# google/TensorNetwork

Hardware: NVIDIA H100
Metric: pairwise contractions/s (higher is better)
Workload: dtype bf16

## Files before the change

include/tnb200.h:

```cpp
#ifndef TNB200_H_
#define TNB200_H_

#include <stdint.h>

#if defined(TNB200_BUILD)
#define TNB200_API __attribute__((visibility("default")))
#else
#define TNB200_API
#endif

#ifdef __cplusplus
extern "C" {
#endif

#define TNB200_MAX_NDIM 16
#define TNB200_ABI_VERSION 1

typedef enum {
  TNB200_OK = 0,
  TNB200_ERR_INVALID = -1,
  TNB200_ERR_DTYPE = -2,
  TNB200_ERR_CUDA = -3,
  TNB200_ERR_UNSUPPORTED = -4,
  TNB200_ERR_NOCONV = -5
// ... 76 lines not shown
                     int32_t axis1, int32_t axis2, void* stream);
TNB200_API int32_t tnb200_diagflat(const tnb200_tensor_t* a, const tnb200_tensor_t* c, int64_t k,
                        void* stream);

TNB200_API int32_t tnb200_svd(const tnb200_tensor_t* a, const tnb200_tensor_t* u, const tnb200_tensor_t* s,
                   const tnb200_tensor_t* vh, int32_t* info_dev, void* stream);
TNB200_API int32_t tnb200_svd_truncation_count(const tnb200_tensor_t* s, int64_t max_singular_values,
                                    int32_t use_error, double max_truncation_error,
                                    int32_t relative, int64_t* keep_dev, void* stream);

TNB200_API int32_t tnb200_eigh(const tnb200_tensor_t* a, const tnb200_tensor_t* w, const tnb200_tensor_t* v,
                               int32_t* info_dev, void* stream);

TNB200_API int32_t tnb200_arnoldi_orth(const tnb200_tensor_t* v, int32_t j, const tnb200_tensor_t* w, void* h_dev,
                                       void* stream);

TNB200_API int32_t tnb200_qr(const tnb200_tensor_t* a, const tnb200_tensor_t* q, const tnb200_tensor_t* r,
                  int32_t non_negative_diagonal, void* stream);

TNB200_API int32_t tnb200_lu_factor(const tnb200_tensor_t* a, const tnb200_tensor_t* lu, int32_t* piv_dev,
                                    int32_t* info_dev, void* stream);
TNB200_API int32_t tnb200_inv(const tnb200_tensor_t* a, const tnb200_tensor_t* x, int32_t* info_dev, void* stream);

TNB200_API int32_t tnb200_blocksparse_tensordot(const void* a_data, const void* b_data, void* c_data,
                                     int32_t dtype, int32_t nsect, const int64_t* dims_dev,
                                     const int64_t* a_map_dev, const int64_t* a_off_dev,
                                     const int64_t* b_map_dev, const int64_t* b_off_dev,
                                     const int64_t* c_map_dev, const int64_t* c_off_dev,
                                     int64_t max_m, int64_t max_n, int32_t conj_b, void* stream);

TNB200_API int32_t tnb200_svd_batched(const void* a_data, int32_t dtype, int32_t nprob, const int64_t* dims_dev,
                                      const int64_t* a_off_dev, void* u_data, const int64_t* u_off_dev, void* s_data,
                                      const int64_t* s_off_dev, void* vh_data, const int64_t* vh_off_dev,
                                      int64_t max_m, int64_t max_n, int32_t* status_dev, void* stream);

TNB200_API int32_t tnb200_blocksparse_maps(int32_t nlegs, const int64_t* dims, const int64_t* charges_dev, const int64_t* leg_off,
                                           const int32_t* order, int32_t partition, int32_t split, int64_t modulus, int64_t shift,
                                           int32_t nbins, const int64_t* tables_dev, int64_t nnz, int64_t* map_dev, void* stream);

TNB200_API int32_t tnb200_gather(const void* src, const int64_t* idx_dev, void* dst, int64_t n, int32_t dtype,
                                 int32_t scatter, void* stream);

typedef struct {
  tnb200_tensor_t a, b, c;
  int32_t naxes, nbatch;
  int32_t axes_a[TNB200_MAX_NDIM], axes_b[TNB200_MAX_NDIM];
  int32_t batch_a[TNB200_MAX_NDIM], batch_b[TNB200_MAX_NDIM];
  int32_t dep_a, dep_b;
} tnb200_chain_step_t;
TNB200_API int32_t tnb200_chain_create(int32_t nsteps, const tnb200_chain_step_t* steps, int32_t* first_unsupported,
                                       void** handle);
TNB200_API int32_t tnb200_chain_launch(void* handle, void* stream);
TNB200_API int32_t tnb200_chain_destroy(void* handle);

TNB200_API int32_t tnb200_thin_run_create(int32_t nsteps, const tnb200_chain_step_t* steps, int32_t* first_unsupported,
                                          void** handle);
TNB200_API int32_t tnb200_thin_run_launch(void* handle, void* stream);
TNB200_API int32_t tnb200_thin_run_destroy(void* handle);

#ifdef __cplusplus
}
#endif
#endif
```

tensornetwork_b200/_lib.py:

```python
import ctypes
import os

MAX_NDIM = 16
LIB_PATH = os.path.join(os.path.dirname(os.path.abspath(__file__)), "lib", "libtnb200.so")

F64, F32, F16, BF16, C64, C128, I32, I64, BOOL = range(9)
OK, ERR_INVALID, ERR_DTYPE, ERR_CUDA, ERR_UNSUPPORTED, ERR_NOCONV = 0, -1, -2, -3, -4, -5
ADD, SUB, MUL, DIV, POW = range(5)
CONJ, SQRT, ABS, NEG, EXP, LOG, SIN, COS, SIGN, REAL, IMAG = range(11)
LT, LE, GT, GE = range(4)
CONJ_A, CONJ_B = 1, 2
MATH_DEFAULT, MATH_STRICT, MATH_SIMT = 0 << 4, 1 << 4, 2 << 4


class TensorDesc(ctypes.Structure):
  _fields_ = [("data", ctypes.c_void_p), ("dtype", ctypes.c_int32), ("ndim", ctypes.c_int32),
              ("shape", ctypes.c_int64 * MAX_NDIM), ("stride", ctypes.c_int64 * MAX_NDIM)]


class ChainStep(ctypes.Structure):
  _fields_ = [("a", TensorDesc), ("b", TensorDesc), ("c", TensorDesc), ("naxes", ctypes.c_int32), ("nbatch", ctypes.c_int32),
              ("axes_a", ctypes.c_int32 * MAX_NDIM), ("axes_b", ctypes.c_int32 * MAX_NDIM),
              ("batch_a", ctypes.c_int32 * MAX_NDIM), ("batch_b", ctypes.c_int32 * MAX_NDIM),
              ("dep_a", ctypes.c_int32), ("dep_b", ctypes.c_int32)]


_P = ctypes.POINTER(TensorDesc)
_i32, _i64, _u64, _dbl, _vp = (ctypes.c_int32, ctypes.c_int64, ctypes.c_uint64, ctypes.c_double,
                               ctypes.c_void_p)
_pi32 = ctypes.POINTER(ctypes.c_int32)

SIGNATURES = {
    "tnb200_last_error": (ctypes.c_char_p, []),
    "tnb200_abi_version": (_i32, []),
    "tnb200_device_info": (_i32, [_pi32, _pi32, _pi32, ctypes.POINTER(_i64)]),
    "tnb200_last_kernel": (ctypes.c_char_p, []),
    "tnb200_launch_count": (_i64, []),
    "tnb200_tensordot": (_i32, [_P, _P, _P, _i32, _pi32, _pi32, _i32, _pi32, _pi32, _i32, _vp]),
    "tnb200_copy": (_i32, [_P, _P, _i32, _vp]),
    "tnb200_binary": (_i32, [_i32, _P, _P, _P, _vp]),
    "tnb200_unary": (_i32, [_i32, _P, _P, _vp]),
    "tnb200_affine_inplace": (_i32, [_P, _dbl, _dbl, _dbl, _dbl, _vp]),
    "tnb200_scale_by_device_scalar": (_i32, [_P, _vp, _i32, _i32, _vp]),
    "tnb200_axpy": (_i32, [_P, _P, _dbl, _dbl, _vp, _dbl, _vp]),
    "tnb200_fill": (_i32, [_P, _dbl, _dbl, _vp]),
    "tnb200_compare": (_i32, [_i32, _P, _P, _P, _vp]),
    "tnb200_index_update": (_i32, [_P, _P, _dbl, _dbl, _vp, _i32, _P, _vp]),
    "tnb200_eye": (_i32, [_P, _i64, _vp]),
    "tnb200_randn": (_i32, [_P, _u64, _vp]),
    "tnb200_uniform": (_i32, [_P, _dbl, _dbl, _u64, _vp]),
    "tnb200_norm": (_i32, [_P, _vp, _vp]),
    "tnb200_dot": (_i32, [_P, _P, _i32, _vp, _vp]),
    "tnb200_sum": (_i32, [_P, _P, _i32, _pi32, _vp]),
    "tnb200_trace": (_i32, [_P, _P, _i64, _i32, _i32, _vp]),
    "tnb200_diagflat": (_i32, [_P, _P, _i64, _vp]),
    "tnb200_svd": (_i32, [_P, _P, _P, _P, _vp, _vp]),
    "tnb200_svd_truncation_count": (_i32, [_P, _i64, _i32, _dbl, _i32, _vp, _vp]),
    "tnb200_eigh": (_i32, [_P, _P, _P, _vp, _vp]),
    "tnb200_arnoldi_orth": (_i32, [_P, _i32, _P, _vp, _vp]),
    "tnb200_qr": (_i32, [_P, _P, _P, _i32, _vp]),
    "tnb200_lu_factor": (_i32, [_P, _P, _vp, _vp, _vp]),
    "tnb200_inv": (_i32, [_P, _P, _vp, _vp]),
    "tnb200_blocksparse_maps": (_i32, [_i32, _vp, _vp, _vp, _vp, _i32, _i32, _i64, _i64, _i32, _vp, _i64, _vp, _vp]),
    "tnb200_svd_batched": (_i32, [_vp, _i32, _i32, _vp, _vp, _vp, _vp, _vp, _vp, _vp, _vp, _i64, _i64, _vp, _vp]),
    "tnb200_gather": (_i32, [_vp, _vp, _vp, _i64, _i32, _i32, _vp]),
    "tnb200_blocksparse_tensordot": (_i32, [_vp, _vp, _vp, _i32, _i32, _vp, _vp, _vp, _vp, _vp,
                                            _vp, _vp, _i64, _i64, _i32, _vp]),
    "tnb200_chain_create": (_i32, [_i32, ctypes.POINTER(ChainStep), _pi32, ctypes.POINTER(_vp)]),
    "tnb200_chain_launch": (_i32, [_vp, _vp]),
    "tnb200_chain_destroy": (_i32, [_vp]),
    "tnb200_thin_run_create": (_i32, [_i32, ctypes.POINTER(ChainStep), _pi32, ctypes.POINTER(_vp)]),
    "tnb200_thin_run_launch": (_i32, [_vp, _vp]),
    "tnb200_thin_run_destroy": (_i32, [_vp]),
}

_lib = None


def load(path=None):
  global _lib
  if _lib is not None:
    return _lib
  path = path or os.environ.get("TNB200_LIB", LIB_PATH)
  if not os.path.exists(path):
    raise OSError("libtnb200.so not found at {} — build it with "
                  "`python -m tensornetwork_b200.build` (there is no CPU fallback)".format(path))
  lib = ctypes.CDLL(path)
  for name, (res, args) in SIGNATURES.items():
    fn = getattr(lib, name)
    fn.restype = res
    fn.argtypes = args
  if lib.tnb200_abi_version() != 1:
    raise OSError("libtnb200.so ABI version mismatch")
  _lib = lib
  return lib


def set_lib(obj):
  global _lib
  _lib = obj


class Tnb200Error(RuntimeError):
  pass


def check(rc):
  if rc == 0:
    return
  msg = _lib.tnb200_last_error()
  msg = msg.decode() if isinstance(msg, bytes) else str(msg)
  if rc == ERR_INVALID:
    raise ValueError(msg)
  if rc == ERR_DTYPE:
    raise TypeError(msg)
  if rc == ERR_UNSUPPORTED:
    raise NotImplementedError(msg)
  raise Tnb200Error("tnb200 status {}: {}".format(rc, msg))
```

tensornetwork_b200/csrc/gemm_wgmma.cu:

```cuda
#include "gemm.cuh"
#include "wgmma.cuh"
#include <cuda.h>
#include <mutex>
#include <vector>

namespace tnb {

__device__ __forceinline__ uint32_t smem_u32(const void* p) { return (uint32_t)__cvta_generic_to_shared(p); }

__device__ __forceinline__ void mbar_init(uint32_t bar, uint32_t count) {
  asm volatile("mbarrier.init.shared::cta.b64 [%0], %1;" ::"r"(bar), "r"(count));
}
__device__ __forceinline__ void mbar_expect_tx(uint32_t bar, uint32_t bytes) {
  asm volatile("mbarrier.arrive.expect_tx.shared::cta.b64 _, [%0], %1;" ::"r"(bar), "r"(bytes) : "memory");
}
__device__ __forceinline__ void mbar_arrive(uint32_t bar) {
  asm volatile("mbarrier.arrive.shared::cta.b64 _, [%0];" ::"r"(bar) : "memory");
}
__device__ __forceinline__ void mbar_wait(uint32_t bar, uint32_t parity) {
  uint32_t done = 0;
#pragma unroll 1
  for (uint32_t it = 0; it < (1u << 28); ++it) {
    asm volatile(
        "{\n\t.reg .pred p;\n\t"
        "mbarrier.try_wait.parity.shared::cta.b64 p, [%1], %2;\n\t"
        "selp.u32 %0, 1, 0, p;\n\t}"
        : "=r"(done) : "r"(bar), "r"(parity) : "memory");
    if (done) return;
  }
  __trap();
}
__device__ __forceinline__ void tma_load_5d(uint32_t dst, const CUtensorMap* map, uint32_t bar, int c0, int c1, int c2, int c3, int c4) {
  asm volatile(
      "cp.async.bulk.tensor.5d.shared::cluster.global.mbarrier::complete_tx::bytes [%0], [%1, {%3, %4, %5, %6, %7}], [%2];"
      ::"r"(dst), "l"(map), "r"(bar), "r"(c0), "r"(c1), "r"(c2), "r"(c3), "r"(c4) : "memory");
}
__device__ __forceinline__ void tma_load_5d_pair(uint32_t dst, const CUtensorMap* map, uint32_t bar,
                                                 int c0, int c1, int c2, int c3, int c4) {
  asm volatile(
      "cp.async.bulk.tensor.5d.shared::cluster.global.mbarrier::complete_tx::bytes.multicast::cluster"
      " [%0], [%1, {%3, %4, %5, %6, %7}], [%2], %8;"
      ::"r"(dst), "l"(map), "r"(bar), "r"(c0), "r"(c1), "r"(c2), "r"(c3), "r"(c4), "h"((uint16_t)0x3) : "memory");
}
__device__ __forceinline__ uint32_t cluster_ctarank() {
  uint32_t r;
  asm volatile("mov.u32 %0, %%cluster_ctarank;" : "=r"(r));
  return r;
}
__device__ __forceinline__ void mbar_arrive_cluster(uint32_t bar, uint32_t cta) {
  asm volatile(
      "{\n\t.reg .b32 remote;\n\t"
      "mapa.shared::cluster.u32 remote, %0, %1;\n\t"
      "mbarrier.arrive.shared::cluster.b64 _, [remote];\n\t}"
      ::"r"(bar), "r"(cta) : "memory");
}
// ... 23 lines not shown
}

struct TcParams {
  int64_t M, N, K, batch;
  int BN, num_kb, stages, out_kind;
  int64_t tiles_m, tiles_n, num_tiles;
  int a_mn, b_mn;
  uint32_t a_fe, a_ke, b_fe, b_ke;
  void* C; int64_t c_sm, c_sb;
  int64_t c_cs;
  int vec_ok;
};

constexpr int kBM = 128;
constexpr int kRowBytes = 128;
constexpr int kThreads = 384;

struct alignas(64) ChainStepDev {
  CUtensorMap tmA, tmB, tmC;
  TcParams p;
  int dep_a, dep_b;
  uint32_t need_a, need_b;
  int tiles_per_sample;
};
struct ChainSeg { long long tile0; int step, sample0, nsamples, pad; };
struct ChainParams {
  const ChainStepDev* steps;
  const ChainSeg* segs;
  uint32_t* done;
  long long num_tiles;
  int nsegs, batch, stages, stage_bytes;
};
constexpr int kConsumerWarps = 8;
constexpr int kChainBN16 = 256, kChainBN32 = 128;
constexpr int kBoxBytes = 64 * 128;
constexpr int kChainStageHalf = 2 * kBoxBytes;

struct KernelArgs {
  CUtensorMap tmA, tmB;
  TcParams p;
  ChainParams cp;
  int stage_bytes;
};

__device__ __forceinline__ uint32_t ld_acquire_u32(const uint32_t* p) {
  uint32_t v;
  asm volatile("ld.acquire.gpu.global.u32 %0, [%1];" : "=r"(v) : "l"(p) : "memory");
  return v;
}
__device__ __forceinline__ void red_release_add_u32(uint32_t* p, uint32_t v) {
  asm volatile("red.release.gpu.global.add.u32 [%0], %1;" ::"l"(p), "r"(v) : "memory");
}
#ifdef TNB200_CHAIN_PHASES
constexpr int kPhases = 6;
constexpr int kPhaseCtas = 1024;
__device__ unsigned long long g_chain_phase[kPhaseCtas * kPhases];
__device__ __forceinline__ unsigned long long phase_clock() {
  unsigned long long t;
  asm volatile("mov.u64 %0, %%globaltimer;" : "=l"(t)::"memory");
  return t;
}
#define TNB_PHASE(...) __VA_ARGS__
#define TNB_PHASE_ADD(slot, v) (g_chain_phase[blockIdx.x * kPhases + (slot)] += (v))
#else
#define TNB_PHASE(...)
#endif

__device__ __forceinline__ void chain_wait(const uint32_t* ctr, uint32_t need) {
#pragma unroll 1
  for (uint32_t it = 0; it < (1u << 24); ++it) {
    if (ld_acquire_u32(ctr) >= need) return;
    __nanosleep(64);
  }
  __trap();
}

struct Tile {
  const TcParams* p;
  const CUtensorMap *ma, *mb;
  const ChainStepDev* sd;
  int bi, mi, ni, step;
  bool live;
};
template <bool CHAIN>
__device__ __forceinline__ void decode_tile(const KernelArgs& a, long long tile, int rank, int& cursor, Tile& t) {
  if (!CHAIN) {
    uint32_t x = (uint32_t)tile;
    const uint32_t tn = (uint32_t)a.p.tiles_n, tm = (uint32_t)a.p.tiles_m;
    t.ni = (int)(x % tn); x /= tn;
    t.mi = (int)(x % tm);
    t.bi = (int)(x / tm);
    t.p = &a.p; t.ma = &a.tmA; t.mb = &a.tmB; t.sd = nullptr; t.step = 0;
    t.live = true;
  } else {
    const ChainParams& cp = a.cp;
    while (cursor + 1 < cp.nsegs && tile >= cp.segs[cursor + 1].tile0) ++cursor;
    const ChainSeg sg = cp.segs[cursor];
    const ChainStepDev* sd = cp.steps + sg.step;
    uint32_t local = (uint32_t)(tile - sg.tile0);
    const uint32_t tn = (uint32_t)sd->p.tiles_n, tm = (uint32_t)sd->p.tiles_m, pm = (tm + 1) / 2;
    t.ni = (int)(local % tn); local /= tn;
    t.mi = 2 * (int)(local % pm) + rank;
    t.bi = sg.sample0 + (int)(local / pm);
    t.step = sg.step;
    t.p = &sd->p; t.ma = &sd->tmA; t.mb = &sd->tmB; t.sd = sd;
    t.live = (uint32_t)t.mi < tm;
  }
// ... 8 lines not shown
    const int m = idx & 31, rest = idx >> 5, kc = rest & 7;
    const int r = (rest >> 3) * 32 + m;
    const bool is_a = r < rows_a;
    const int rr = is_a ? r : r - rows_a;
    const uint32_t src = staging + (is_a ? 0u : a_bytes) + (uint32_t)(rr >> 5) * 4096u;
    const uint32_t dst = stage + (is_a ? 0u : a_bytes) + (uint32_t)rr * 128u + (uint32_t)((kc ^ (rr & 7)) << 4);
    uint32_t v[4];
#pragma unroll
    for (int i = 0; i < 4; ++i) {
      const int k = kc * 4 + i;
      const uint32_t addr = src + (uint32_t)k * 128u + (uint32_t)((((m >> 2) ^ (k & 7)) << 4) | ((m & 3) << 2));
      asm volatile("ld.shared.b32 %0, [%1];" : "=r"(v[i]) : "r"(addr) : "memory");
    }
    asm volatile("st.shared.v4.b32 [%0], {%1, %2, %3, %4};" ::"r"(dst), "r"(v[0]), "r"(v[1]), "r"(v[2]), "r"(v[3]) : "memory");
  }
  asm volatile("fence.proxy.async.shared::cta;" ::: "memory");
}

template <int KIND, int BN, int TA, int TB>
__device__ __forceinline__ void mma_k(float* d, uint64_t a, uint64_t b, uint32_t acc) {
  if constexpr (KIND == 2) {
    if constexpr (BN == 64) wgmma_n64_tf32(d, a, b, acc);
    else if constexpr (BN == 128) wgmma_n128_tf32(d, a, b, acc);
    else wgmma_n256_tf32(d, a, b, acc);
  } else if constexpr (KIND == 0) {
    if constexpr (BN == 64) wgmma_n64_bf16<TA, TB>(d, a, b, acc);
    else if constexpr (BN == 128) wgmma_n128_bf16<TA, TB>(d, a, b, acc);
    else wgmma_n256_bf16<TA, TB>(d, a, b, acc);
  } else {
    if constexpr (BN == 64) wgmma_n64_f16<TA, TB>(d, a, b, acc);
    else if constexpr (BN == 128) wgmma_n128_f16<TA, TB>(d, a, b, acc);
    else wgmma_n256_f16<TA, TB>(d, a, b, acc);
  }
}

template <bool PAIR>
__device__ __forceinline__ void release_slot(uint32_t bar) {
  if constexpr (PAIR) { mbar_arrive_cluster(bar, 0); mbar_arrive_cluster(bar, 1); }
  else mbar_arrive(bar);
}

__device__ __forceinline__ void drainloop(int S, uint32_t bar_base, int num_kb, int lane, int& s, uint32_t& ph) {
#pragma unroll 1
  for (int kb = 0; kb < num_kb; ++kb) {
    mbar_wait(bar_base + 8u * s, ph);
    __syncwarp();
    if (lane == 0) release_slot<true>(bar_base + 8u * (S + s));
    if (++s == S) { s = 0; ph ^= 1; }
  }
}

template <int KIND, int BN, int TA, int TB, bool PAIR>
__device__ __forceinline__ void mainloop(float* d, uint8_t* smem, int stage_bytes, int S, uint32_t bar_base, int num_kb,
                                         int a_mn, int b_mn, int wg, int ctid, int lane, int& s, uint32_t& ph) {
  constexpr int BK = kRowBytes / (KIND == 2 ? 4 : 2);
  constexpr uint32_t a_lbo = TA ? BK * kRowBytes : 16u, b_lbo = TB ? BK * kRowBytes : 16u;
  constexpr uint32_t a_kstep = TA ? 16u * kRowBytes : 32u, b_kstep = TB ? 16u * kRowBytes : 32u;
  int prev = -1;
  for (int kb = 0; kb < num_kb; ++kb) {
    TNB_PHASE(const unsigned long long tw = phase_clock();)
    mbar_wait(bar_base + 8u * s, ph);
    TNB_PHASE(if (ctid == 0) TNB_PHASE_ADD(1, phase_clock() - tw);)
    const uint32_t sa = smem_u32(smem + (size_t)s * stage_bytes);
    if (KIND == 2 && (a_mn || b_mn)) {
      transpose_stage_tf32(sa, a_mn, b_mn, BN, ctid);
      consumers_sync();
    }
    const uint32_t sa_wg = sa + (uint32_t)wg * 64u * kRowBytes;
    const uint32_t sb = sa + kBM * kRowBytes;
    wg_fence();
#pragma unroll
    for (int k = 0; k < 4; ++k)
      mma_k<KIND, BN, TA, TB>(d, gmma_desc(sa_wg + k * a_kstep, a_lbo, 1024u), gmma_desc(sb + k * b_kstep, b_lbo, 1024u),
                              (kb > 0 || k > 0) ? 1u : 0u);
    wg_commit();
    if (prev >= 0) {
      wg_wait<1>();
      __syncwarp();
      if (lane == 0) release_slot<PAIR>(bar_base + 8u * (S + prev));
    }
    prev = s;
    if (++s == S) { s = 0; ph ^= 1; }
  }
  wg_wait<0>();
  __syncwarp();
  if (lane == 0) release_slot<PAIR>(bar_base + 8u * (S + prev));
}

__device__ __forceinline__ void store_one(const TcParams& p, int64_t off, float v) {
  if (p.out_kind == 2) ((float*)p.C)[off] = v;
  else if (p.out_kind == 0) ((__nv_bfloat16*)p.C)[off] = __float2bfloat16_rn(v);
  else ((__half*)p.C)[off] = __float2half_rn(v);
}
__device__ __forceinline__ void store_pair(const TcParams& p, int64_t off, float v0, float v1) {
  if (p.out_kind == 2) *(float2*)((float*)p.C + off) = make_float2(v0, v1);
  else if (p.out_kind == 0) *(__nv_bfloat162*)((__nv_bfloat16*)p.C + off) = __floats2bfloat162_rn(v0, v1);
  else *(__half2*)((__half*)p.C + off) = __floats2half2_rn(v0, v1);
}

template <int KIND, int BN, bool CHAIN>
__global__ void __launch_bounds__(kThreads, 1)
gemm_wgmma_kernel(const __grid_constant__ KernelArgs args) {
  constexpr int ES = KIND == 2 ? 4 : 2;
  constexpr int BK = kRowBytes / ES;
  constexpr int CHUNK = kRowBytes / ES;
  constexpr int A_BYTES = kBM * kRowBytes;
  constexpr int B_BYTES = BN * kRowBytes;
  extern __shared__ __align__(1024) uint8_t smem_raw[];
  uint8_t* smem = (uint8_t*)(((uintptr_t)smem_raw + 1023) & ~(uintptr_t)1023);
  const int STAGE_BYTES = args.stage_bytes;
  const int S = CHAIN ? args.cp.stages : args.p.stages;
  const long long num_tiles = CHAIN ? args.cp.num_tiles : args.p.num_tiles;
  constexpr int STAGE_HALF = kChainStageHalf;
  const uint32_t staging = smem_u32(smem + (size_t)S * STAGE_BYTES);
  uint64_t* bars = (uint64_t*)(smem + (size_t)S * STAGE_BYTES + (CHAIN ? 2 * STAGE_HALF : 0));
// ... 3 lines not shown
  auto staged_bar = [&](int wg) { return bar_base + 8u * (2 * S + wg); };
  auto freed_bar = [&](int wg) { return bar_base + 8u * (2 * S + 2 + wg); };

  const int warp = threadIdx.x >> 5, lane = threadIdx.x & 31;
  TNB_PHASE(const unsigned long long t_start = phase_clock();)
  if (threadIdx.x == 0) {
    if (!CHAIN) {
      asm volatile("prefetch.tensormap [%0];" ::"l"(&args.tmA) : "memory");
      asm volatile("prefetch.tensormap [%0];" ::"l"(&args.tmB) : "memory");
    }
    for (int s = 0; s < S; ++s) {
      mbar_init(full_bar(s), 1);
      mbar_init(empty_bar(s), (CHAIN ? 2 : 1) * kConsumerWarps);
    }
    if (CHAIN)
      for (int wg = 0; wg < 2; ++wg) { mbar_init(staged_bar(wg), 4); mbar_init(freed_bar(wg), 1); }
    asm volatile("fence.mbarrier_init.release.cluster;" ::: "memory");
  }
  if constexpr (CHAIN) cluster_sync();
  else __syncthreads();
  const int rank = CHAIN ? (int)cluster_ctarank() : 0;
  const long long first = CHAIN ? blockIdx.x / 2 : blockIdx.x, step = CHAIN ? gridDim.x / 2 : gridDim.x;

  if (warp == 0) {
    constexpr int B_SPLIT = CHAIN ? 2 : 1;
    int s = 0; uint32_t ph = 0;
    int cursor = 0;
    for (long long tile = first; tile < num_tiles; tile += step) {
      Tile t;
      decode_tile<CHAIN>(args, tile, rank, cursor, t);
      const TcParams& p = *t.p;
      const int a_mn = p.a_mn, b_mn = p.b_mn;
      const int nA = t.live ? (a_mn ? kBM / CHUNK : 1) : 0;
      const int nB = b_mn ? BN / CHUNK / B_SPLIT : 1;
      const bool mine = lane < nA + nB;
      const bool is_a = lane < nA;
      const bool mn = is_a ? (a_mn != 0) : (b_mn != 0);
      const int c = is_a ? lane : rank * nB + lane - nA;
      const int fbox = mn ? CHUNK : (is_a ? kBM : BN / B_SPLIT);
      const uint32_t fe = is_a ? p.a_fe : p.b_fe, ke = is_a ? p.a_ke : p.b_ke;
      const CUtensorMap* map = is_a ? t.ma : t.mb;
      uint32_t dst_off = (is_a ? 0u : (uint32_t)A_BYTES) + (uint32_t)(c * fbox * kRowBytes);
      if (KIND == 2 && mn) dst_off += A_BYTES + B_BYTES;
      const int f = (is_a ? t.mi * kBM : t.ni * BN) + c * fbox;
      const int f_in = fe ? (int)((uint32_t)f % fe) : f, f_out = fe ? (int)((uint32_t)f / fe) : 0;
      const uint32_t tx_bytes = (t.live ? A_BYTES : 0) + B_BYTES;
      const int num_kb = p.num_kb;
      if (CHAIN) {
        if (lane == 0) {
          TNB_PHASE(const unsigned long long tw = phase_clock();)
          const ChainStepDev* sd = t.sd;
          if (sd->dep_a >= 0) chain_wait(args.cp.done + (size_t)sd->dep_a * args.cp.batch + t.bi, sd->need_a);
          if (sd->dep_b >= 0) chain_wait(args.cp.done + (size_t)sd->dep_b * args.cp.batch + t.bi, sd->need_b);
          TNB_PHASE(TNB_PHASE_ADD(0, phase_clock() - tw);)
        }
        __syncwarp();
        asm volatile("fence.proxy.async;" ::: "memory");
      }
      int k_in = 0, k_out = 0;
      for (int kb = 0; kb < num_kb; ++kb) {
        mbar_wait(empty_bar(s), ph ^ 1);
        const uint32_t full = full_bar(s);
        if (lane == 0) mbar_expect_tx(full, tx_bytes);
        __syncwarp();
        if (mine) {
          const uint32_t dst = smem_u32(smem + (size_t)s * STAGE_BYTES) + dst_off;
          const int x0 = mn ? f_in : k_in, x1 = mn ? k_in : f_in, x2 = mn ? k_out : f_out, x3 = mn ? f_out : k_out;
          if (CHAIN && !is_a) tma_load_5d_pair(dst, map, full, x0, x1, x2, x3, t.bi);
          else                tma_load_5d(dst, map, full, x0, x1, x2, x3, t.bi);
        }
        k_in += BK;
        if (ke && (uint32_t)k_in >= ke) { k_in = 0; ++k_out; }
        if (++s == S) { s = 0; ph ^= 1; }
      }
    }
  } else if (warp >= 4) {
    const int ctid = threadIdx.x - 128;
    const int wg = ctid >> 7;
    const int wt = ctid & 127;
    int s = 0; uint32_t ph = 0;
    uint32_t eph = 0;
    int cursor = 0;
    float d[BN / 2];
    for (long long tile = first; tile < num_tiles; tile += step) {
      Tile t;
      decode_tile<CHAIN>(args, tile, rank, cursor, t);
      const TcParams& p = *t.p;
      const int a_mn = p.a_mn, b_mn = p.b_mn, num_kb = p.num_kb;
      if (CHAIN && !t.live) {
        drainloop(S, bar_base, num_kb, lane, s, ph);
        continue;
      }
      TNB_PHASE(const unsigned long long tk = phase_clock();)
      if constexpr (KIND == 2) {
        mainloop<KIND, BN, 0, 0, CHAIN>(d, smem, STAGE_BYTES, S, bar_base, num_kb, a_mn, b_mn, wg, ctid, lane, s, ph);
      } else {
        if (a_mn && b_mn) mainloop<KIND, BN, 1, 1, CHAIN>(d, smem, STAGE_BYTES, S, bar_base, num_kb, a_mn, b_mn, wg, ctid, lane, s, ph);
        else if (a_mn) mainloop<KIND, BN, 1, 0, CHAIN>(d, smem, STAGE_BYTES, S, bar_base, num_kb, a_mn, b_mn, wg, ctid, lane, s, ph);
        else if (b_mn) mainloop<KIND, BN, 0, 1, CHAIN>(d, smem, STAGE_BYTES, S, bar_base, num_kb, a_mn, b_mn, wg, ctid, lane, s, ph);
        else mainloop<KIND, BN, 0, 0, CHAIN>(d, smem, STAGE_BYTES, S, bar_base, num_kb, a_mn, b_mn, wg, ctid, lane, s, ph);
      }
      TNB_PHASE(const unsigned long long te = phase_clock(); if (ctid == 0) TNB_PHASE_ADD(2, te - tk);)
      const int r0 = (wt >> 5) * 16 + (lane >> 2);
      if constexpr (CHAIN) {
        constexpr int J_PER_PASS = BN / 8 * STAGE_HALF / (4 * kBoxBytes);
        const uint32_t half = staging + (uint32_t)wg * STAGE_HALF;
#pragma unroll
        for (int pass = 0; pass < 4 * kBoxBytes / STAGE_HALF; ++pass) {
          mbar_wait(freed_bar(wg), eph ^ 1);
#pragma unroll
          for (int jj = 0; jj < J_PER_PASS; ++jj) {
            const int j = pass * J_PER_PASS + jj;
            const uint32_t colb = (uint32_t)(8 * j + 2 * (lane & 3)) * ES - (uint32_t)pass * STAGE_HALF / 64;
#pragma unroll
            for (int h = 0; h < 2; ++h) {
              const uint32_t r = (uint32_t)(r0 + 8 * h);
              const uint32_t addr = half + (colb >> 7) * kBoxBytes + r * 128u + ((((colb >> 4) & 7) ^ (r & 7)) << 4) + (colb & 15);
              const float v0 = d[4 * j + 2 * h], v1 = d[4 * j + 2 * h + 1];
              if constexpr (KIND == 2) {
                asm volatile("st.shared.v2.f32 [%0], {%1, %2};" ::"r"(addr), "f"(v0), "f"(v1) : "memory");
              } else {
                uint32_t u;
                if constexpr (KIND == 0) { __nv_bfloat162 x = __floats2bfloat162_rn(v0, v1); u = *(uint32_t*)&x; }
                else { __half2 x = __floats2half2_rn(v0, v1); u = *(uint32_t*)&x; }
                asm volatile("st.shared.b32 [%0], %1;" ::"r"(addr), "r"(u) : "memory");
              }
            }
          }
          asm volatile("fence.proxy.async.shared::cta;" ::: "memory");
          __syncwarp();
          if (lane == 0) mbar_arrive(staged_bar(wg));
          eph ^= 1;
        }
        TNB_PHASE(if (ctid == 0) { TNB_PHASE_ADD(3, phase_clock() - te); TNB_PHASE_ADD(5, 1); })
        continue;
      }
      const int64_t row0 = (int64_t)t.mi * kBM + wg * 64 + r0;
      const int64_t n0 = (int64_t)t.ni * BN + 2 * (lane & 3);
      const int64_t cb = (int64_t)t.bi * p.c_sb;
#pragma unroll
      for (int h = 0; h < 2; ++h) {
        const int64_t row = row0 + 8 * h;
        if (row < p.M) {
#pragma unroll
          for (int j = 0; j < BN / 8; ++j) {
            const int64_t col = n0 + 8 * j;
            const float v0 = d[4 * j + 2 * h], v1 = d[4 * j + 2 * h + 1];
            if (p.c_cs == 1) {
              const int64_t off = cb + row * p.c_sm + col;
              if (p.vec_ok && col + 1 < p.N) store_pair(p, off, v0, v1);
              else {
                if (col < p.N) store_one(p, off, v0);
                if (col + 1 < p.N) store_one(p, off + 1, v1);
              }
            } else {
              const int64_t off = cb + row * p.c_sm + col * p.c_cs;
              if (col < p.N) store_one(p, off, v0);
              if (col + 1 < p.N) store_one(p, off + p.c_cs, v1);
            }
          }
        }
      }
    }
    TNB_PHASE(if (ctid == 0) TNB_PHASE_ADD(4, phase_clock() - t_start);)
  } else if (CHAIN && warp == 1 && lane == 0) {
    int cursor = 0;
    uint32_t sph = 0;
    for (long long tile = first; tile < num_tiles; tile += step) {
      Tile t;
      decode_tile<CHAIN>(args, tile, rank, cursor, t);
      if (!t.live) continue;
      const CUtensorMap* mc = &t.sd->tmC;
#pragma unroll 1
      for (int pass = 0; pass < 4 * kBoxBytes / STAGE_HALF; ++pass) {
#pragma unroll 1
        for (int wg = 0; wg < 2; ++wg) {
          mbar_wait(staged_bar(wg), sph);
          for (int b = 0; b < STAGE_HALF / kBoxBytes; ++b) {
            const int box = pass * (STAGE_HALF / kBoxBytes) + b;
            tma_store_3d(mc, staging + (uint32_t)(wg * STAGE_HALF + b * kBoxBytes), t.ni * BN + box * (128 / ES),
                         t.mi * kBM + wg * 64, t.bi);
          }
          bulk_commit();
          bulk_wait_read_all();
          mbar_arrive(freed_bar(wg));
        }
        sph ^= 1;
      }
      bulk_wait_all();
      asm volatile("fence.proxy.async.global;" ::: "memory");
      red_release_add_u32(args.cp.done + (size_t)t.step * args.cp.batch + t.bi, 1u);
    }
  }
  if constexpr (CHAIN) cluster_sync();
}

typedef CUresult (*EncodeTiledFn)(CUtensorMap*, CUtensorMapDataType, cuuint32_t, void*, const cuuint64_t*,
                                  const cuuint64_t*, const cuuint32_t*, const cuuint32_t*, CUtensorMapInterleave,
                                  CUtensorMapSwizzle, CUtensorMapL2promotion, CUtensorMapFloatOOBfill);
static EncodeTiledFn get_encode() {
  static EncodeTiledFn fn = nullptr;
  static std::once_flag once;
  std::call_once(once, []() {
    void* p = nullptr;
    cudaDriverEntryPointQueryResult q;
    if (cudaGetDriverEntryPoint("cuTensorMapEncodeTiled", &p, cudaEnableDefault, &q) == cudaSuccess &&
        q == cudaDriverEntryPointSuccess)
      fn = (EncodeTiledFn)p;
  });
  return fn;
}

static int es_of(int dt) { return dt == TNB200_F32 ? 4 : 2; }
static int kind_of(int dt) { return dt == TNB200_BF16 ? 0 : (dt == TNB200_F16 ? 1 : 2); }

static int view_major(int dtype, const OperandView& v, int64_t ext_f, int64_t ext_k, int64_t batch) {
  if (dtype != TNB200_F32 && dtype != TNB200_F16 && dtype != TNB200_BF16) return -1;
// ... 184 lines not shown
    t.c_sm = g.c_sn; t.c_sn = g.c_sm;
    return gemm_wgmma(t, st);
  }
  KernelArgs args;
  memset(&args, 0, sizeof(args));
  {
    TcPrep prep;
    int rc = tc_prepare(g, false, prep);
    if (rc) return rc;
    args.tmA = prep.tmA; args.tmB = prep.tmB; args.p = prep.p; args.stage_bytes = prep.stage_bytes;
  }
  const int kind = kind_of(g.dtype);
  KernelFn fn = kernel_of(kind, args.p.BN, false);
  static bool attr_set[3][3] = {};
  const int bi = args.p.BN == 64 ? 0 : (args.p.BN == 128 ? 1 : 2);
  if (!attr_set[kind][bi]) {
    int rc = raise_smem(fn);
    if (rc) return rc;
    attr_set[kind][bi] = true;
  }
  const int64_t sms = num_sms();
  const int64_t grid = args.p.num_tiles < sms ? args.p.num_tiles : sms;
  fn<<<(unsigned)grid, kThreads, smem_of(args.p.stages, args.stage_bytes), st>>>(args);
  TNB_LAUNCH_CHECK();
  count_launch();
  set_kernel_name(kind == 0 ? "wgmma_bf16" : (kind == 1 ? "wgmma_f16" : "wgmma_tf32"));
  return 0;
}

struct ChainHandle {
  ChainStepDev* d_steps = nullptr;
  ChainSeg* d_segs = nullptr;
  uint32_t* d_done = nullptr;
  KernelArgs args;
  int kind = 0, nsteps = 0;
  size_t smem = 0, done_bytes = 0;
  unsigned grid = 0;
};

struct PairLaunch {
  cudaLaunchAttribute attr;
  cudaLaunchConfig_t cfg;
  PairLaunch(unsigned grid, size_t smem, cudaStream_t st) {
    memset(&attr, 0, sizeof(attr));
    attr.id = cudaLaunchAttributeClusterDimension;
    attr.val.clusterDim.x = 2; attr.val.clusterDim.y = 1; attr.val.clusterDim.z = 1;
    memset(&cfg, 0, sizeof(cfg));
    cfg.gridDim = dim3(grid); cfg.blockDim = dim3(kThreads); cfg.dynamicSmemBytes = smem; cfg.stream = st;
    cfg.attrs = &attr; cfg.numAttrs = 1;
  }
  PairLaunch(const PairLaunch&) = delete;
};

int gemm_chain_create(int nsteps, const GemmProblem* probs, const int* dep_a, const int* dep_b, int* first_unsupported,
                      void** handle) {
  *handle = nullptr;
  if (nsteps < 1) return TNB200_ERR_INVALID;
  auto reject = [&](int i, int rc) { if (first_unsupported) *first_unsupported = i; return rc; };
  for (int i = 0; i < nsteps; ++i) {
    const GemmProblem& g = probs[i];
    if (g.M < 128 || g.N < 128 || g.batch != probs[0].batch || g.dtype != probs[0].dtype)
      return reject(i, TNB200_ERR_UNSUPPORTED);
  }
  const int dtype = probs[0].dtype;
  const int64_t batch = probs[0].batch;
  std::vector<ChainStepDev> steps(nsteps);
  int max_stage = 0;
  std::vector<int64_t> step_bytes(nsteps), out_bytes(nsteps);
  for (int i = 0; i < nsteps; ++i) {
    const GemmProblem& g = probs[i];
    if (g.conjA || g.conjB || g.swapped) return reject(i, TNB200_ERR_UNSUPPORTED);
    if (g.dtype != TNB200_F32 && g.dtype != TNB200_F16 && g.dtype != TNB200_BF16) return reject(i, TNB200_ERR_UNSUPPORTED);
    if (g.c_sn != 1 || g.M >= (1LL << 31) || g.N >= (1LL << 31) || g.K >= (1LL << 31)) return reject(i, TNB200_ERR_UNSUPPORTED);
    if (dep_a[i] >= i || dep_b[i] >= i) return TNB200_ERR_INVALID;
    TcPrep prep;
    int rc = tc_prepare(g, true, prep);
    if (rc) return reject(i, rc);
    ChainStepDev& sd = steps[i];
    memset(&sd, 0, sizeof(sd));
    rc = encode_output(&sd.tmC, g);
    if (rc) return reject(i, rc);
    sd.tmA = prep.tmA; sd.tmB = prep.tmB; sd.p = prep.p;
    sd.dep_a = dep_a[i]; sd.dep_b = dep_b[i];
    sd.tiles_per_sample = (int)(prep.p.tiles_m * prep.p.tiles_n);
    if (prep.stage_bytes > max_stage) max_stage = prep.stage_bytes;
    step_bytes[i] = (g.M * g.K + g.N * g.K + g.M * g.N) * es_of(dtype);
    out_bytes[i] = g.M * g.N * es_of(dtype);
  }
  for (int i = 0; i < nsteps; ++i) {
    if (steps[i].dep_a >= 0) steps[i].need_a = (uint32_t)steps[steps[i].dep_a].tiles_per_sample;
    if (steps[i].dep_b >= 0) steps[i].need_b = (uint32_t)steps[steps[i].dep_b].tiles_per_sample;
  }
  const int kind = kind_of(dtype);
  KernelFn fn = kernel_of(kind, 0, true);
  {
    static bool attr_set[3] = {};
    if (!attr_set[kind]) {
      int rc = raise_smem(fn);
      if (rc) return rc;
      attr_set[kind] = true;
    }
  }
  const int staging = 2 * kChainStageHalf;
  int stages = (227 * 1024 - 1024 - staging - 256) / max_stage;
  if (stages > 8) stages = 8;
  if (stages < 2) return TNB200_ERR_UNSUPPORTED;
  const size_t smem = smem_of(stages, max_stage) + staging + 4 * 8;
  int clusters = 0;
  {
    PairLaunch pl(2 * num_sms(), smem, nullptr);
    if (cudaOccupancyMaxActiveClusters(&clusters, (void*)fn, &pl.cfg) != cudaSuccess) {
      cudaGetLastError();
      clusters = 0;
    }
  }
  if (clusters < 1) return TNB200_ERR_UNSUPPORTED;
  std::vector<int> pps(nsteps);
  for (int i = 0; i < nsteps; ++i) pps[i] = (int)(steps[i].p.tiles_n * ((steps[i].p.tiles_m + 1) / 2));
  auto env_int = [](const char* name, int dflt) { const char* e = getenv(name); return e ? atoi(e) : dflt; };
  int min_pps = pps[0];
  for (int i = 1; i < nsteps; ++i) if (pps[i] < min_pps) min_pps = pps[i];
  if (batch * min_pps < clusters && !env_int("TNB200_CHAIN_FORCE", 0))
    return TNB200_ERR_UNSUPPORTED;
  int l2 = 0;
  {
    int dev = 0;
    if (cudaGetDevice(&dev) != cudaSuccess || cudaDeviceGetAttribute(&l2, cudaDevAttrL2CacheSize, dev) != cudaSuccess) {
      cudaGetLastError();
      l2 = 0;
    }
  }
  int g_wave = 1;
  std::vector<int> last_reader(nsteps, -1);
  for (int i = 0; i < nsteps; ++i) {
    for (const int d : {dep_a[i], dep_b[i]}) {
      if (d < 0) continue;
      last_reader[d] = i;
      int64_t gap = 0;
      for (int j = d; j < i; ++j) gap += pps[j];
      const int g = (int)((clusters + gap - 1) / gap);
      if (g > g_wave) g_wave = g;
    }
  }
  int64_t live_bytes = 0;
  for (int i = 0; i < nsteps; ++i) {
    int64_t live = step_bytes[i];
    for (int j = 0; j < i; ++j)
      if (last_reader[j] > i && dep_a[i] != j && dep_b[i] != j) live += out_bytes[j];
    if (live > live_bytes) live_bytes = live;
  }
  const int g_l2 = (int)(l2 / live_bytes);
  int G = env_int("TNB200_CHAIN_G", g_wave > g_l2 ? g_wave : g_l2);
  if (G < 1) G = 1;
  const int64_t rounds = (batch + G - 1) / G;
  std::vector<ChainSeg> segs;
  long long tile0 = 0;
  for (int64_t r = 0; r < rounds; ++r) {
    const int64_t r0 = batch * r / rounds, r1 = batch * (r + 1) / rounds;
    for (int i = 0; i < nsteps; ++i) {
      ChainSeg sg;
      sg.tile0 = tile0; sg.step = i; sg.sample0 = (int)r0; sg.nsamples = (int)(r1 - r0); sg.pad = 0;
      segs.push_back(sg);
      tile0 += (long long)(r1 - r0) * pps[i];
    }
  }
  ChainHandle* h = new ChainHandle();
  h->kind = kind;
  h->nsteps = nsteps;
  h->done_bytes = sizeof(uint32_t) * (size_t)nsteps * (size_t)batch;
  cudaError_t e = cudaMalloc(&h->d_steps, sizeof(ChainStepDev) * steps.size());
  if (e == cudaSuccess) e = cudaMalloc(&h->d_segs, sizeof(ChainSeg) * segs.size());
  if (e == cudaSuccess) e = cudaMalloc(&h->d_done, h->done_bytes);
  if (e == cudaSuccess) e = cudaMemcpy(h->d_steps, steps.data(), sizeof(ChainStepDev) * steps.size(), cudaMemcpyHostToDevice);
  if (e == cudaSuccess) e = cudaMemcpy(h->d_segs, segs.data(), sizeof(ChainSeg) * segs.size(), cudaMemcpyHostToDevice);
  if (e != cudaSuccess) {
    set_error("chain: device table allocation failed: %s", cudaGetErrorString(e));
    cudaFree(h->d_steps); cudaFree(h->d_segs); cudaFree(h->d_done);
    delete h;
    return TNB200_ERR_CUDA;
  }
  memset(&h->args, 0, sizeof(h->args));
  ChainParams& cp = h->args.cp;
  cp.steps = h->d_steps; cp.segs = h->d_segs; cp.done = h->d_done;
  cp.num_tiles = tile0; cp.nsegs = (int)segs.size(); cp.batch = (int)batch;
  cp.stages = stages; cp.stage_bytes = max_stage;
  h->args.stage_bytes = max_stage;
  h->smem = smem;
  h->grid = (unsigned)(2 * (tile0 < clusters ? tile0 : clusters));
  *handle = h;
  return 0;
}

int gemm_chain_launch(void* handle, cudaStream_t st) {
  ChainHandle* h = (ChainHandle*)handle;
  if (!h) return TNB200_ERR_INVALID;
  TNB_CHECK_CUDA(cudaMemsetAsync(h->d_done, 0, h->done_bytes, st));
  PairLaunch pl(h->grid, h->smem, st);
  TNB_CHECK_CUDA(cudaLaunchKernelEx(&pl.cfg, kernel_of(h->kind, 0, true), h->args));
  count_launch();
  set_kernel_name(h->kind == 2 ? "wgmma_chain_tf32" : "wgmma_chain_16");
  return 0;
}

int gemm_chain_destroy(void* handle) {
  ChainHandle* h = (ChainHandle*)handle;
  if (!h) return 0;
  cudaFree(h->d_steps); cudaFree(h->d_segs); cudaFree(h->d_done);
  delete h;
  return 0;
}

}

#ifdef TNB200_CHAIN_PHASES
extern "C" TNB200_API int32_t tnb200_chain_phases(unsigned long long* out, int32_t reset) {
  if (cudaMemcpyFromSymbol(out, tnb::g_chain_phase, sizeof(tnb::g_chain_phase)) != cudaSuccess) return TNB200_ERR_CUDA;
  if (reset) {
    void* p = nullptr;
    if (cudaGetSymbolAddress(&p, tnb::g_chain_phase) != cudaSuccess || cudaMemset(p, 0, sizeof(tnb::g_chain_phase)) != cudaSuccess)
      return TNB200_ERR_CUDA;
  }
  return 0;
}
#endif
```

Baseline: 1.139 million.

## Factor chain scheduler, cap round size, add interleaved rounds option

Moves chain segment scheduling into a reusable `chain_schedule` routine, also exposed through a C API. By default the per-round sample count is now capped at twice the wave-covering gap instead of growing to fill L2. An optional `TNB200_CHAIN_W` setting interleaves several rounds in flight, with a binary search on modelled L2 live bytes to pick the round count. Phase profiling is also split by dependency class. The cap gives more, smaller rounds, which may improve L2 locality but costs more dependency waits per sample.

```diff
diff --git a/include/tnb200.h b/include/tnb200.h
--- a/include/tnb200.h
+++ b/include/tnb200.h
@@ -152,6 +152,10 @@
                                        void** handle);
 TNB200_API int32_t tnb200_chain_launch(void* handle, void* stream);
 TNB200_API int32_t tnb200_chain_destroy(void* handle);
+TNB200_API int32_t tnb200_chain_schedule(int32_t nsteps, const int32_t* pairs, const int32_t* dep_a, const int32_t* dep_b,
+                                         const int64_t* step_bytes, const int64_t* out_bytes, int64_t batch,
+                                         int32_t clusters, int64_t l2_bytes, int32_t G, int32_t W, int32_t force,
+                                         int64_t* segs, int32_t max_segs, int32_t* info, int64_t* model);
 
 TNB200_API int32_t tnb200_thin_run_create(int32_t nsteps, const tnb200_chain_step_t* steps, int32_t* first_unsupported,
                                           void** handle);
diff --git a/tensornetwork_b200/_lib.py b/tensornetwork_b200/_lib.py
--- a/tensornetwork_b200/_lib.py
+++ b/tensornetwork_b200/_lib.py
@@ -69,6 +69,8 @@
     "tnb200_chain_create": (_i32, [_i32, ctypes.POINTER(ChainStep), _pi32, ctypes.POINTER(_vp)]),
     "tnb200_chain_launch": (_i32, [_vp, _vp]),
     "tnb200_chain_destroy": (_i32, [_vp]),
+    "tnb200_chain_schedule": (_i32, [_i32, _pi32, _pi32, _pi32, ctypes.POINTER(_i64), ctypes.POINTER(_i64), _i64, _i32,
+                                     _i64, _i32, _i32, _i32, ctypes.POINTER(_i64), _i32, _pi32, ctypes.POINTER(_i64)]),
     "tnb200_thin_run_create": (_i32, [_i32, ctypes.POINTER(ChainStep), _pi32, ctypes.POINTER(_vp)]),
     "tnb200_thin_run_launch": (_i32, [_vp, _vp]),
     "tnb200_thin_run_destroy": (_i32, [_vp]),
diff --git a/tensornetwork_b200/csrc/gemm_wgmma.cu b/tensornetwork_b200/csrc/gemm_wgmma.cu
--- a/tensornetwork_b200/csrc/gemm_wgmma.cu
+++ b/tensornetwork_b200/csrc/gemm_wgmma.cu
@@ -1,6 +1,8 @@
 #include "gemm.cuh"
 #include "wgmma.cuh"
 #include <cuda.h>
+#include <algorithm>
+#include <cstdio>
 #include <mutex>
 #include <vector>
 
@@ -130,7 +132,9 @@
   asm volatile("red.release.gpu.global.add.u32 [%0], %1;" ::"l"(p), "r"(v) : "memory");
 }
 #ifdef TNB200_CHAIN_PHASES
-constexpr int kPhases = 6;
+constexpr int kPhases = 16;
+constexpr int kPhFirst = 4, kPhRest = 8, kPhLoop = 9, kPhEpi = 10, kPhLife = 11, kPhTiles = 12;
+__device__ __forceinline__ int phase_class(const ChainStepDev* sd) { return (sd->dep_a >= 0 ? 1 : 0) + (sd->dep_b >= 0 ? 2 : 0); }
 constexpr int kPhaseCtas = 1024;
 __device__ unsigned long long g_chain_phase[kPhaseCtas * kPhases];
 __device__ __forceinline__ unsigned long long phase_clock() {
@@ -245,7 +249,8 @@
 
 template <int KIND, int BN, int TA, int TB, bool PAIR>
 __device__ __forceinline__ void mainloop(float* d, uint8_t* smem, int stage_bytes, int S, uint32_t bar_base, int num_kb,
-                                         int a_mn, int b_mn, int wg, int ctid, int lane, int& s, uint32_t& ph) {
+                                         int a_mn, int b_mn, int wg, int ctid, int lane, int& s, uint32_t& ph
+                                         TNB_PHASE(, int cls)) {
   constexpr int BK = kRowBytes / (KIND == 2 ? 4 : 2);
   constexpr uint32_t a_lbo = TA ? BK * kRowBytes : 16u, b_lbo = TB ? BK * kRowBytes : 16u;
   constexpr uint32_t a_kstep = TA ? 16u * kRowBytes : 32u, b_kstep = TB ? 16u * kRowBytes : 32u;
@@ -253,7 +258,7 @@
   for (int kb = 0; kb < num_kb; ++kb) {
     TNB_PHASE(const unsigned long long tw = phase_clock();)
     mbar_wait(bar_base + 8u * s, ph);
-    TNB_PHASE(if (ctid == 0) TNB_PHASE_ADD(1, phase_clock() - tw);)
+    TNB_PHASE(if (ctid == 0) TNB_PHASE_ADD(kb == 0 ? kPhFirst + cls : kPhRest, phase_clock() - tw);)
     const uint32_t sa = smem_u32(smem + (size_t)s * stage_bytes);
     if (KIND == 2 && (a_mn || b_mn)) {
       transpose_stage_tf32(sa, a_mn, b_mn, BN, ctid);
@@ -363,7 +368,7 @@
           const ChainStepDev* sd = t.sd;
           if (sd->dep_a >= 0) chain_wait(args.cp.done + (size_t)sd->dep_a * args.cp.batch + t.bi, sd->need_a);
           if (sd->dep_b >= 0) chain_wait(args.cp.done + (size_t)sd->dep_b * args.cp.batch + t.bi, sd->need_b);
-          TNB_PHASE(TNB_PHASE_ADD(0, phase_clock() - tw);)
+          TNB_PHASE(TNB_PHASE_ADD(phase_class(sd), phase_clock() - tw);)
         }
         __syncwarp();
         asm volatile("fence.proxy.async;" ::: "memory");
@@ -402,16 +407,16 @@
         drainloop(S, bar_base, num_kb, lane, s, ph);
         continue;
       }
-      TNB_PHASE(const unsigned long long tk = phase_clock();)
+      TNB_PHASE(const unsigned long long tk = phase_clock(); const int cls = CHAIN ? phase_class(t.sd) : 0;)
       if constexpr (KIND == 2) {
-        mainloop<KIND, BN, 0, 0, CHAIN>(d, smem, STAGE_BYTES, S, bar_base, num_kb, a_mn, b_mn, wg, ctid, lane, s, ph);
+        mainloop<KIND, BN, 0, 0, CHAIN>(d, smem, STAGE_BYTES, S, bar_base, num_kb, a_mn, b_mn, wg, ctid, lane, s, ph TNB_PHASE(, cls));
       } else {
-        if (a_mn && b_mn) mainloop<KIND, BN, 1, 1, CHAIN>(d, smem, STAGE_BYTES, S, bar_base, num_kb, a_mn, b_mn, wg, ctid, lane, s, ph);
-        else if (a_mn) mainloop<KIND, BN, 1, 0, CHAIN>(d, smem, STAGE_BYTES, S, bar_base, num_kb, a_mn, b_mn, wg, ctid, lane, s, ph);
-        else if (b_mn) mainloop<KIND, BN, 0, 1, CHAIN>(d, smem, STAGE_BYTES, S, bar_base, num_kb, a_mn, b_mn, wg, ctid, lane, s, ph);
-        else mainloop<KIND, BN, 0, 0, CHAIN>(d, smem, STAGE_BYTES, S, bar_base, num_kb, a_mn, b_mn, wg, ctid, lane, s, ph);
+        if (a_mn && b_mn) mainloop<KIND, BN, 1, 1, CHAIN>(d, smem, STAGE_BYTES, S, bar_base, num_kb, a_mn, b_mn, wg, ctid, lane, s, ph TNB_PHASE(, cls));
+        else if (a_mn) mainloop<KIND, BN, 1, 0, CHAIN>(d, smem, STAGE_BYTES, S, bar_base, num_kb, a_mn, b_mn, wg, ctid, lane, s, ph TNB_PHASE(, cls));
+        else if (b_mn) mainloop<KIND, BN, 0, 1, CHAIN>(d, smem, STAGE_BYTES, S, bar_base, num_kb, a_mn, b_mn, wg, ctid, lane, s, ph TNB_PHASE(, cls));
+        else mainloop<KIND, BN, 0, 0, CHAIN>(d, smem, STAGE_BYTES, S, bar_base, num_kb, a_mn, b_mn, wg, ctid, lane, s, ph TNB_PHASE(, cls));
       }
-      TNB_PHASE(const unsigned long long te = phase_clock(); if (ctid == 0) TNB_PHASE_ADD(2, te - tk);)
+      TNB_PHASE(const unsigned long long te = phase_clock(); if (ctid == 0) TNB_PHASE_ADD(kPhLoop, te - tk);)
       const int r0 = (wt >> 5) * 16 + (lane >> 2);
       if constexpr (CHAIN) {
         constexpr int J_PER_PASS = BN / 8 * STAGE_HALF / (4 * kBoxBytes);
@@ -443,7 +448,7 @@
           if (lane == 0) mbar_arrive(staged_bar(wg));
           eph ^= 1;
         }
-        TNB_PHASE(if (ctid == 0) { TNB_PHASE_ADD(3, phase_clock() - te); TNB_PHASE_ADD(5, 1); })
+        TNB_PHASE(if (ctid == 0) { TNB_PHASE_ADD(kPhEpi, phase_clock() - te); TNB_PHASE_ADD(kPhTiles + cls, 1); })
         continue;
       }
       const int64_t row0 = (int64_t)t.mi * kBM + wg * 64 + r0;
@@ -473,7 +478,7 @@
         }
       }
     }
-    TNB_PHASE(if (ctid == 0) TNB_PHASE_ADD(4, phase_clock() - t_start);)
+    TNB_PHASE(if (ctid == 0) TNB_PHASE_ADD(kPhLife, phase_clock() - t_start);)
   } else if (CHAIN && warp == 1 && lane == 0) {
     int cursor = 0;
     uint32_t sph = 0;
@@ -764,6 +769,108 @@
   PairLaunch(const PairLaunch&) = delete;
 };
 
+struct ChainSchedule {
+  int G = 0, W = 0, rounds = 0;
+  int64_t min_gap = 0, live = 0;
+  std::vector<ChainSeg> segs;
+};
+
+static int64_t chain_rounds(int64_t batch, int G, int W) { return ((batch + G - 1) / G + W - 1) / W * W; }
+
+static bool chain_sequence(int nsteps, const int* pps, const int* dep_a, const int* dep_b, const int64_t* run_bytes,
+                           const int64_t* held_bytes, int64_t batch, int64_t R, int W, ChainSchedule& s) {
+  if (R < 1 || R > batch || R % W) return false;
+  const int64_t per = R / W, ticks = W - 1 + per * nsteps;
+  s.G = (int)((batch + R - 1) / R); s.W = W; s.rounds = (int)R;
+  s.min_gap = INT64_MAX; s.live = 0;
+  s.segs.clear();
+  std::vector<long long> pos((size_t)nsteps * R);
+  std::vector<int64_t> tick((size_t)nsteps * R);
+  auto samples = [&](int64_t r) { return batch * (r + 1) / R - batch * r / R; };
+  long long tile0 = 0;
+  for (int64_t t = 0; t < ticks; ++t) {
+    for (int k = 0; k < W; ++k) {
+      const int64_t u = t - k;
+      if (u < 0 || u / nsteps >= per) continue;
+      const int64_t r = u / nsteps * W + k;
+      const int i = (int)(u % nsteps);
+      const int64_t n = samples(r);
+      ChainSeg sg;
+      sg.tile0 = tile0; sg.step = i; sg.sample0 = (int)(batch * r / R); sg.nsamples = (int)n; sg.pad = 0;
+      s.segs.push_back(sg);
+      pos[(size_t)i * R + r] = tile0; tick[(size_t)i * R + r] = t;
+      for (const int d : {dep_a[i], dep_b[i]})
+        if (d >= 0 && tick[(size_t)d * R + r] >= W - 1 && t <= ticks - W) {
+          const int64_t gap = tile0 - pos[(size_t)d * R + r];
+          if (gap < s.min_gap) s.min_gap = gap;
+        }
+      int64_t live = n * run_bytes[i];
+      for (int k2 = 0; k2 < W; ++k2) {
+        const int64_t u2 = t - k2;
+        if (k2 == k || u2 < 0 || u2 / nsteps >= per) continue;
+        const int next = (int)(u2 % nsteps) + (k2 < k ? 1 : 0);
+        live += samples(u2 / nsteps * W + k2) * held_bytes[next];
+      }
+      if (live > s.live) s.live = live;
+      tile0 += (long long)n * pps[i];
+    }
+  }
+  return true;
+}
+
+static int chain_schedule(int nsteps, const int* pps, const int* dep_a, const int* dep_b, const int64_t* step_bytes,
+                          const int64_t* out_bytes, int64_t batch, int clusters, int64_t l2, int G, int W, bool force,
+                          ChainSchedule& out) {
+  if (nsteps < 1 || batch < 1 || clusters < 1 || W < 0) return TNB200_ERR_INVALID;
+  for (int i = 0; i < nsteps; ++i)
+    if (pps[i] < 1 || dep_a[i] >= i || dep_b[i] >= i || step_bytes[i] < 0 || out_bytes[i] < 0) return TNB200_ERR_INVALID;
+  int min_pps = pps[0];
+  for (int i = 1; i < nsteps; ++i) if (pps[i] < min_pps) min_pps = pps[i];
+  if (batch * min_pps < clusters && !force)
+    return TNB200_ERR_UNSUPPORTED;
+  int g_wave = 1, g_wave2 = 1;
+  std::vector<int> last_reader(nsteps, -1);
+  for (int i = 0; i < nsteps; ++i) {
+    for (const int d : {dep_a[i], dep_b[i]}) {
+      if (d < 0) continue;
+      last_reader[d] = i;
+      int64_t gap = 0;
+      for (int j = d; j < i; ++j) gap += pps[j];
+      const int g = (int)((clusters + gap - 1) / gap), g2 = (int)((2 * clusters + gap - 1) / gap);
+      if (g > g_wave) g_wave = g;
+      if (g2 > g_wave2) g_wave2 = g2;
+    }
+  }
+  std::vector<int64_t> run_bytes(nsteps), held_bytes(nsteps + 1, 0);
+  int64_t live_bytes = 0;
+  for (int i = 0; i < nsteps; ++i) {
+    run_bytes[i] = step_bytes[i];
+    for (int j = 0; j < i; ++j)
+      if (last_reader[j] > i && dep_a[i] != j && dep_b[i] != j) run_bytes[i] += out_bytes[j];
+    if (run_bytes[i] > live_bytes) live_bytes = run_bytes[i];
+    for (int j = 0; j < i; ++j)
+      if (last_reader[j] >= i) held_bytes[i] += out_bytes[j];
+  }
+  const int64_t g_l2 = live_bytes > 0 ? l2 / live_bytes : batch;
+  const int64_t g_rule = std::max<int64_t>(g_wave, std::min<int64_t>(g_wave2, g_l2));
+  const int G1 = G > 0 ? G : (int)std::max<int64_t>(1, std::min<int64_t>(g_rule, batch));
+  const auto seq = [&](int64_t R, int w, ChainSchedule& o) {
+    return chain_sequence(nsteps, pps, dep_a, dep_b, run_bytes.data(), held_bytes.data(), batch, R, w, o);
+  };
+  const auto fit = [&](int w, ChainSchedule& o) {
+    int64_t lo = 1, hi = batch / w, best = 0;
+    while (lo <= hi) {
+      const int64_t m = (lo + hi) / 2;
+      if (seq(m * w, w, o) && o.live <= l2) { best = m; hi = m - 1; } else lo = m + 1;
+    }
+    return best > 0 && seq(best * w, w, o);
+  };
+  const bool ok = W <= 1 || G > 0 ? seq(chain_rounds(batch, G1, W > 1 ? W : 1), W > 1 ? W : 1, out)
+                                  : fit(W, out) || seq(batch / W * W, W, out);
+  if (!ok) return TNB200_ERR_INVALID;
+  return 0;
+}
+
 int gemm_chain_create(int nsteps, const GemmProblem* probs, const int* dep_a, const int* dep_b, int* first_unsupported,
                       void** handle) {
   *handle = nullptr;
@@ -829,11 +936,6 @@
   if (clusters < 1) return TNB200_ERR_UNSUPPORTED;
   std::vector<int> pps(nsteps);
   for (int i = 0; i < nsteps; ++i) pps[i] = (int)(steps[i].p.tiles_n * ((steps[i].p.tiles_m + 1) / 2));
-  auto env_int = [](const char* name, int dflt) { const char* e = getenv(name); return e ? atoi(e) : dflt; };
-  int min_pps = pps[0];
-  for (int i = 1; i < nsteps; ++i) if (pps[i] < min_pps) min_pps = pps[i];
-  if (batch * min_pps < clusters && !env_int("TNB200_CHAIN_FORCE", 0))
-    return TNB200_ERR_UNSUPPORTED;
   int l2 = 0;
   {
     int dev = 0;
@@ -842,40 +944,20 @@
       l2 = 0;
     }
   }
-  int g_wave = 1;
-  std::vector<int> last_reader(nsteps, -1);
-  for (int i = 0; i < nsteps; ++i) {
-    for (const int d : {dep_a[i], dep_b[i]}) {
-      if (d < 0) continue;
-      last_reader[d] = i;
-      int64_t gap = 0;
-      for (int j = d; j < i; ++j) gap += pps[j];
-      const int g = (int)((clusters + gap - 1) / gap);
-      if (g > g_wave) g_wave = g;
-    }
-  }
-  int64_t live_bytes = 0;
-  for (int i = 0; i < nsteps; ++i) {
-    int64_t live = step_bytes[i];
-    for (int j = 0; j < i; ++j)
-      if (last_reader[j] > i && dep_a[i] != j && dep_b[i] != j) live += out_bytes[j];
-    if (live > live_bytes) live_bytes = live;
-  }
-  const int g_l2 = (int)(l2 / live_bytes);
-  int G = env_int("TNB200_CHAIN_G", g_wave > g_l2 ? g_wave : g_l2);
-  if (G < 1) G = 1;
-  const int64_t rounds = (batch + G - 1) / G;
-  std::vector<ChainSeg> segs;
-  long long tile0 = 0;
-  for (int64_t r = 0; r < rounds; ++r) {
-    const int64_t r0 = batch * r / rounds, r1 = batch * (r + 1) / rounds;
-    for (int i = 0; i < nsteps; ++i) {
-      ChainSeg sg;
-      sg.tile0 = tile0; sg.step = i; sg.sample0 = (int)r0; sg.nsamples = (int)(r1 - r0); sg.pad = 0;
-      segs.push_back(sg);
-      tile0 += (long long)(r1 - r0) * pps[i];
-    }
-  }
+  auto env_int = [](const char* name, int dflt) { const char* e = getenv(name); return e ? atoi(e) : dflt; };
+  ChainSchedule sched;
+  const int rc_s = chain_schedule(nsteps, pps.data(), dep_a, dep_b, step_bytes.data(), out_bytes.data(), batch, clusters,
+                                  l2, env_int("TNB200_CHAIN_G", 0), env_int("TNB200_CHAIN_W", 0),
+                                  env_int("TNB200_CHAIN_FORCE", 0) != 0, sched);
+  if (rc_s) return rc_s;
+#ifdef TNB200_CHAIN_PHASES
+  fprintf(stderr, "chain schedule: %d steps, %d samples, rounds of <= %d samples (%d rounds), %d in flight, "
+          "smallest dependency gap %lld pairs = %.2f waves of %d clusters, modelled L2 live %.1f MB of %.1f MB\n",
+          nsteps, (int)batch, sched.G, sched.rounds, sched.W, (long long)sched.min_gap,
+          (double)sched.min_gap / clusters, clusters, sched.live / 1048576.0, l2 / 1048576.0);
+#endif
+  const std::vector<ChainSeg>& segs = sched.segs;
+  const long long tile0 = segs.back().tile0 + (long long)segs.back().nsamples * pps[segs.back().step];
   ChainHandle* h = new ChainHandle();
   h->kind = kind;
   h->nsteps = nsteps;
@@ -924,6 +1006,28 @@
 
 }
 
+extern "C" TNB200_API int32_t tnb200_chain_schedule(int32_t nsteps, const int32_t* pairs, const int32_t* dep_a,
+                                                    const int32_t* dep_b, const int64_t* step_bytes,
+                                                    const int64_t* out_bytes, int64_t batch, int32_t clusters,
+                                                    int64_t l2_bytes, int32_t G, int32_t W, int32_t force,
+                                                    int64_t* segs, int32_t max_segs, int32_t* info, int64_t* model) {
+  if (nsteps < 1 || !pairs || !dep_a || !dep_b || !step_bytes || !out_bytes || !info || !model) return TNB200_ERR_INVALID;
+  tnb::ChainSchedule s;
+  const int rc = tnb::chain_schedule(nsteps, pairs, dep_a, dep_b, step_bytes, out_bytes, batch, clusters, l2_bytes, G, W,
+                                     force != 0, s);
+  if (rc) return rc;
+  info[0] = (int32_t)s.segs.size(); info[1] = s.G; info[2] = s.W; info[3] = s.rounds;
+  model[0] = s.min_gap; model[1] = s.live;
+  if (segs) {
+    if (max_segs < (int32_t)s.segs.size()) return TNB200_ERR_INVALID;
+    for (size_t k = 0; k < s.segs.size(); ++k) {
+      segs[4 * k] = s.segs[k].tile0; segs[4 * k + 1] = s.segs[k].step;
+      segs[4 * k + 2] = s.segs[k].sample0; segs[4 * k + 3] = s.segs[k].nsamples;
+    }
+  }
+  return 0;
+}
+
 #ifdef TNB200_CHAIN_PHASES
 extern "C" TNB200_API int32_t tnb200_chain_phases(unsigned long long* out, int32_t reset) {
   if (cudaMemcpyFromSymbol(out, tnb::g_chain_phase, sizeof(tnb::g_chain_phase)) != cudaSuccess) return TNB200_ERR_CUDA;
```

Result: no change. 1.153 million, median of 6 (+1.2%).
